# RoboEden/flatland-marl

Hardware: AMD Instinct MI355X
Metric: agent-steps/sec (batched envs) + tree-obs build ms/step (higher is better)
Workload: dtype int32; 1 GPU; cfg2: 256 envs x 30x30 / 20 agents / 3 cities (Round-2 Test_2); envs_per_gpu=256, agents=20, obs=cutils(31 nodes, pred 500) + upstream tree depth 2 (pred 30), actions=counter-hash uniform 0..4 generated on device, auto-reset at episode end, distinct_maps=8, dm_rebuild=at commit only, parallelism=envs sharded over 1 GPU(s), metrics all-reduce only, launch=one host call per kernel launch

## Files before the change

### flatland_marl_amd/csrc/fl_obs_body.h

```cpp
#pragma once
#include "fl_obs_trees.h"

__device__ __forceinline__ int obs_env_of_workgroup(const FlObsScratch &S) { return __builtin_amdgcn_readfirstlane(S.order ? S.order[blockIdx.x] : (int)blockIdx.x); }

template <bool CUTILS, int VAR, int STAGE, int MERGED = 0, int FIX = 0, bool UP = true>
__device__ __forceinline__ void obs_body(const FlDev &d, const FlObsScratch &S, const ObsArgs &P_launch) {
    using FixT = ObsFixed<FIX != 0 ? FIX : 1>;
    ObsArgs P_local = P_launch;
    if (FIX != 0) {
        P_local.max_nodes = FixT::max_nodes; P_local.pred_depth = FixT::pred_depth; P_local.tree_pred = FixT::shape.tree_pred;
        P_local.tshift = obs_fixed_tshift<FIX != 0 ? FIX : 1>(d.A);
        if (FixT::max_depth != 0) {
            P_local.max_depth = FixT::max_depth;
            P_local.n_tree_nodes = FixT::max_depth == 2 ? 21 : 85;
        }
    }
    const ObsArgs &P = P_local;
    constexpr bool TAB_LDS = (VAR & 1) != 0, WL_HBM = (VAR & 2) != 0;
    const int b = MERGED == 1 ? (int)blockIdx.x : obs_env_of_workgroup(S), tid = threadIdx.x,
              nt = MERGED == 3 ? 512 : (FIX != 0 || MERGED == 1 || MERGED == 2) ? OBS_NT : (int)blockDim.x;
    const int A = (FIX != 0 && FixT::agents != 0) ? FixT::agents : d.A, R = d.R[b], NS = R * 4, K = d.K[b], U = d.U[b];
    const int Rcap = d.Rcap, Scap = Rcap * 4;
    const int lane = tid & 63, wave = tid >> 6;

// ... 590 lines not shown
                    cutils_pass_a<OBS_CAP_C, TEAM>(X, d, P, b, team_id, have, grp, gl,
                                  merged ? merged_table_c(wave_scr, min(team_id, ROUND - 1)) : wave_scr + min(team_id, min((nt >> 6) * 2, A)) * (N_WORDS_C * OBS_CAP_C),
                                  a_vpos, a_pos, a_dir, a_state, a_speed, a_tslot, (float)T,
                                  a_raw ? a_raw[(have ? team_id : 0) * 8 + 1] : d.spk[b * A + (have ? team_id : 0)],
                                  a_raw ? a_raw[(have ? team_id : 0) * 8 + 2] : d.malf[b * A + (have ? team_id : 0)], node_base, levels);
                    if (gl == 0 && have) { team_meta[64 + team_id] = node_base; team_meta[192 + team_id] = levels; }
                };
                if (p_compact_t) hoisted(std::integral_constant<int, 16>());
                else hoisted(std::integral_constant<int, 32>());
            }
#ifdef FL_OBS_TIMING
            if (lane == 0) {
                atomicMax((unsigned long long *)&X.dbg[19], (unsigned long long)wall_clock64());
                atomicMax((unsigned long long *)&X.dbg[23], (unsigned long long)((long long)wall_clock64() - t_pa0));
            }
#endif
            drain_jobs();
        }
#ifdef FL_OBS_TIMING
        if (lane == 0) atomicMax((unsigned long long *)&X.dbg[22], (unsigned long long)wall_clock64());
#endif
        if (bk && !bk_lds) {
            __syncthreads();
            for (int i = wave; i < A; i += (nt >> 6)) {
                if (lab && lab[i] < 0) continue;
                const uint16_t *path = S.path + ((size_t)b * A + i) * OBS_PRED_CAP;
                const int lp = a_lp[i];
                const int tpc = a_tpc[i], tlast = X.Tn - 1;
                for (int k0 = lane; k0 <= lp; k0 += 256) {
                    uint32_t wv[4];
#pragma unroll
                    for (int q = 0; q < 4; q++) wv[q] = path[min(k0 + 64 * q, lp)];
#pragma unroll
                    for (int q = 0; q < 4; q++) {
                        const int k = k0 + 64 * q;
                        if (k > lp) break;
                        const int key = key_of(X, (int)(wv[q] >> 2));
                        const int tlo = k == 0 ? 0 : (k - 1) * tpc + 1, span = k == 0 ? 1 : tpc;
                        const int thi = (k == lp || tlo + span - 1 >= tlast) ? tlast : tlo + span - 1;
                        const int b1 = min(tlo >> bk_shift, bk_nb - 1), b2 = min(thi >> bk_shift, bk_nb - 1);
                        for (int bb = b1; bb <= b2; bb++) {
                            const int kb = bb * (K + 1) + key + 1;
                            atomicAdd(&bkc[kb >> 1], (kb & 1) ? 0x10000u : 1u);
                        }
                    }
                }
            }
        }
        } else if (!reuse) {
            for (int i = tid; i < A; i += nt) {
                const int n_c = a_n[i];
                const int n_py = (n_c - 1 < pred_depth) ? n_c : pred_depth;
                const int horizon = (X.Tn - 1) / a_tpc[i];
                a_lp[i] = (uint16_t)max(0, min(n_py - 1, horizon));
            }
            __syncthreads();
            for (int i = wave; i < A; i += (nt >> 6)) {
                const uint16_t *path = S.path + ((size_t)b * A + i) * OBS_PRED_CAP;
                const int lp = a_lp[i];
                for (int k = lane; k <= lp; k += 64) atomicAdd(&csr[key_of(X, (int)(path[k] >> 2))], 1);
            }
        }
        __syncthreads();
        OBS_STAMP(3);
        const bool bk_major = bk && !bk_lds;
        if (!reuse && !bk_major) {
            const int chunk = (K + 1 + nt - 1) / nt;
            const int lo = min(tid * chunk, K + 1), hi = min(lo + chunk, K + 1);
            int sum = 0;
            int longest = 0;
            for (int k = lo; k < hi; k++) {
                sum += dual ? (csr[k] | (csr2[k] << 16)) : csr[k];
                longest = max(longest, dual ? max(csr[k], csr2[k]) : csr[k]);
            }
            if (longest > CF_DIRECT && !bk) misc[11] = 1;
            partial[tid] = sum;
            __syncthreads();
            if (wave == 0) {
                constexpr int PER = OBS_NT / 64;
                const int per = nt >> 6;
                int loc[PER], tot = 0;
#pragma unroll
                for (int q = 0; q < PER; q++) { loc[q] = q < per ? partial[lane * per + q] : 0; tot += loc[q]; }
                int incl = tot;
#pragma unroll
                for (int off = 1; off < 64; off <<= 1) { const int v = __shfl_up(incl, off); if (lane >= off) incl += v; }
                int run = incl - tot;
#pragma unroll
                for (int q = 0; q < PER; q++) { if (q < per) partial[lane * per + q] = run; run += loc[q]; }
            }
            __syncthreads();
            int run = partial[tid];
            if (dual) {
                for (int k = lo; k < hi; k++) {
                    const int v = csr[k] | (csr2[k] << 16);
                    csr[k] = run & 0xFFFF; csr2[k] = (int)((unsigned)run >> 16);
                    run += v;
                }
                if (hi == K + 1 && lo < hi) { misc[2] = run & 0xFFFF; misc[3] = (int)((unsigned)run >> 16); }
            } else {
                for (int k = lo; k < hi; k++) { const int v = csr[k]; csr[k] = run; run += v; }
                if (hi == K + 1 && lo < hi) misc[2] = run;
            }
        }
        if (bk_major) {
            uint16_t *c16 = reinterpret_cast<uint16_t *>(bkc);
            const int K1 = K + 1, n = K1 * bk_nb;
            {
                int most = 0;
                for (int key = tid; key < K; key += nt) {
                    int prev = 0;
                    for (int bb = 0; bb < bk_nb; bb++) { const int c = c16[bb * K1 + key + 1]; most = max(most, prev + c); prev = c; }
                }
                if (most > CF_DIRECT) misc[11] = 1;
            }
            const int chunk = (n + nt - 1) / nt;
            const int lo = min(tid * chunk, n), hi = min(lo + chunk, n);
            int sum = 0;
            for (int k = lo; k < hi; k++) sum += c16[k];
            partial[tid] = sum;
            __syncthreads();
            if (wave == 0) {
                constexpr int PER = OBS_NT / 64;
                const int per = nt >> 6;
                int loc[PER], tot = 0;
#pragma unroll
                for (int q = 0; q < PER; q++) { loc[q] = q < per ? partial[lane * per + q] : 0; tot += loc[q]; }
                int incl = tot;
#pragma unroll
                for (int off = 1; off < 64; off <<= 1) { const int v = __shfl_up(incl, off); if (lane >= off) incl += v; }
                int run = incl - tot;
#pragma unroll
                for (int q = 0; q < PER; q++) { if (q < per) partial[lane * per + q] = run; run += loc[q]; }
            }
            __syncthreads();
            {
                int run = partial[tid];
                for (int k = lo; k < hi; k++) {
                    if (k % K1 == 0) misc[12 + k / K1] = run;
                    run += c16[k];
                }
                if (hi == n && lo < hi) misc[2] = run;
            }
            __syncthreads();
            {
                int run = partial[tid], row = lo / K1, rbase = lo < n ? misc[12 + row] : 0, next = (row + 1) * K1;
                for (int k = lo; k < hi; k++) {
                    if (k == next) { row++; rbase = misc[12 + row]; next += K1; }
                    const int c = c16[k];
                    c16[k] = (uint16_t)(run - rbase);
                    run += c;
                }
            }
        }
        __syncthreads();
        if (reuse) {
            csr = csr2; X.csr_end = csr2; X.items_lds = items2;
            X.tmask = p_use_tmask ? tmaskb : nullptr;
            if (!X.tmask) { X.wl_occ_cap = wl_entries; X.wl_cf = X.wl_occ + X.wl_occ_cap; X.wl_cf_cap = 0; }
        }
        if (bk_lds) {
            for (int key = tid; key < K; key += nt) {
                uint32_t *w4 = bkc + key * (bk_w / 2);
                uint32_t run = 0, prev = 0, most = 0;
                for (int q = 0; q < bk_nb / 2; q++) {
                    const uint32_t v = w4[q], c0 = v & 0xFFFFu, c1 = v >> 16;
                    most = max(most, max(prev + c0 + c1, c0 + c1));
                    prev = c0 + c1;
                    w4[q] = run | ((run + c0) << 16);
                    run += c0 + c1;
                }
                if (bk_lds) {
                    const uint32_t ve = w4[bk_nb / 2];
                    w4[bk_nb / 2] = run | (ve & 0xFFFF0000u);
                    most += ve & 0xFFFFu;
                }
                if (most > CF_DIRECT) misc[11] = 1;
            }
            __syncthreads();
        }
#ifdef FL_OBS_TIMING
        if (STAGE != 2) { __syncthreads(); if (tid == 0) P.dbg[(size_t)b * 64 + 56] = (long long)wall_clock64(); }
#endif
        const bool fit = items_lds != nullptr && misc[2] <= L_FIELD(items_cap);
        const bool dual_fill = dual && misc[3] <= L_FIELD(items2_cap);
        if (dual && tid == 0) misc[4] = dual_fill ? 1 : 0;
        if (merged && UP && !dual_fill) atomicCAS(&d.err[b], 0, FL_ERR_CAPACITY);
        if (fit && !reuse) { csr_items = items_lds; X.items_lds = items_lds; }
        constexpr int FU = 4;
#ifdef OBS_NO_LEAN_FILL
        constexpr bool LEAN_FILL = false;
#else
        constexpr bool LEAN_FILL = MERGED == 1;
#endif
        uint32_t pfv[FU] = {0, 0, 0, 0}, pfn[FU] = {0, 0, 0, 0}, pfp[FU] = {0, 0, 0, 0};
        auto prefetch = [&](int ia) __attribute__((always_inline)) {
            if (reuse || ia >= A) return;
            const uint16_t *pth = S.path + ((size_t)b * A + ia) * OBS_PRED_CAP;
            const int lpn = a_lp[ia];
#pragma unroll
            for (int q = 0; q < FU; q++) {
                const int k = min(lane + 64 * q, lpn);
                pfv[q] = pth[k]; pfn[q] = pth[min(k + 1, lpn)]; pfp[q] = pth[max(k - 1, 0)];
            }
        };
        if (bk_major) {
            const int K1 = K + 1, tlast = X.Tn - 1;
            uint16_t *pre16 = reinterpret_cast<uint16_t *>(partial);
            uint16_t *klo16 = pre16 + ((A + 2) & ~1);
            for (int bb = 0; bb < bk_nb; bb++) {
                const int t0 = bb << bk_shift, t1 = bb == bk_nb - 1 ? tlast : min(t0 + (1 << bk_shift) - 1, tlast);
                if (t0 > tlast) break;
                const int gbase = misc[12 + bb];
                for (int ia = tid; ia < A; ia += nt) {
                    const int lp = a_lp[ia], tpc = a_tpc[ia];
                    const int k_lo = min((t0 + tpc - 1) / tpc, lp);
                    const int k_hi = min(t1 >= 1 ? (t1 - 1) / tpc + 1 : 0, lp);
                    klo16[ia] = (uint16_t)k_lo;
                    pre16[ia + 1] = (lab && lab[ia] < 0) ? (uint16_t)0 : (uint16_t)(k_hi - k_lo + 1);
                }
                if (tid == 0) pre16[0] = 0;
                __syncthreads();
                if (wave == 0) {
                    const int per = (A + 63) >> 6, a_lo = min(lane * per, A), a_hi = min(a_lo + per, A);
                    int sum = 0;
                    for (int ia = a_lo; ia < a_hi; ia++) sum += pre16[ia + 1];
                    int incl = sum;
#pragma unroll
                    for (int off = 1; off < 64; off <<= 1) { const int v = __shfl_up(incl, off); if (lane >= off) incl += v; }
                    int run = incl - sum;
                    for (int ia = a_lo; ia < a_hi; ia++) { run += pre16[ia + 1]; pre16[ia + 1] = (uint16_t)run; }
                }
                __syncthreads();
                const int total = pre16[A];
                uint32_t nv = 0, nn = 0, np = 0;
                int n_i = 0, n_k = 0;
                auto request = [&](int t) __attribute__((always_inline)) {
                    if (t >= total) return;
                    int lo_a = 0, hi_a = A - 1;
                    while (lo_a < hi_a) {
                        const int mid = (lo_a + hi_a + 1) >> 1;
                        if ((int)pre16[mid] <= t) lo_a = mid; else hi_a = mid - 1;
                    }
                    n_i = lo_a;
                    n_k = (int)klo16[lo_a] + (t - (int)pre16[lo_a]);
                    const uint16_t *pth = S.path + ((size_t)b * A + lo_a) * OBS_PRED_CAP;
                    const int lp = a_lp[lo_a];
                    nv = pth[n_k]; nn = pth[min(n_k + 1, lp)]; np = pth[max(n_k - 1, 0)];
                };
                request(tid);
                for (int t = tid; t < total; t += nt) {
                    const int i = n_i, k = n_k;
                    const uint32_t w = nv, wnx = nn, wpv = np;
                    request(t + nt);
                    const int lp = a_lp[i], tpc = a_tpc[i];
                    const int tlo = k == 0 ? 0 : (k - 1) * tpc + 1, span = k == 0 ? 1 : tpc;
                    const bool to_end = k == lp || tlo + span - 1 >= tlast;
                    const int thi = to_end ? tlast : tlo + span - 1;
                    const int b1 = min(tlo >> bk_shift, bk_nb - 1), b2 = min(thi >> bk_shift, bk_nb - 1);
                    if (bb < b1 || bb > b2) continue;
                    const int key = key_of(X, (int)(w >> 2));
                    if (X.tmask && bb == b1) {
                        const int m1 = tb_of(tlo, X.tshift), m2 = tb_of(thi, X.tshift);
                        atomicOr(&tmask[key], ((2ull << m2) - 1ull) & ~((1ull << m1) - 1ull));
                    }
                    const uint32_t dnext = k < lp ? (wnx & 3u) : (w & 3u), dprev = k > 0 ? (wpv & 3u) : (w & 3u);
                    const uint32_t item = IT_MAKE(lab ? (int)lab[i] : i, tlo, to_end, span, dprev, dnext, w & 3u);
                    const int kb = bb * K1 + key + 1;
                    const uint32_t old = atomicAdd(&bkc[kb >> 1], (kb & 1) ? 0x10000u : 1u);
                    csr_items[gbase + (int)((kb & 1) ? (old >> 16) : (old & 0xFFFFu))] = item;
                }
                __syncthreads();
            }
        }
        prefetch(bk_major ? A : wave);
        for (int i = wave; !reuse && !bk_major && i < A; i += (nt >> 6)) {
            const uint16_t *path = S.path + ((size_t)b * A + i) * OBS_PRED_CAP;
            const int lp = (lab && lab[i] < 0) ? -1 : (int)a_lp[i], tpc = a_tpc[i], tlast = X.Tn - 1;
            const int lp2 = dual_fill ? (int)a_lp2[i] : -1, tpc2 = dual_fill ? (int)a_tpc2[i] : 1;
            uint32_t wv[FU], wnx[FU], wpv[FU];
#pragma unroll
            for (int q = 0; q < FU; q++) { wv[q] = pfv[q]; wnx[q] = pfn[q]; wpv[q] = pfp[q]; }
            prefetch(i + (nt >> 6));
            for (int k0 = lane; k0 <= lp; k0 += 64 * FU) {
            if (k0 != lane) {
#pragma unroll
                for (int q = 0; q < FU; q++) {
                    const int k = min(k0 + 64 * q, lp);
                    wv[q] = path[k]; wnx[q] = path[min(k + 1, lp)]; wpv[q] = path[max(k - 1, 0)];
                }
            }
#pragma unroll
            for (int q = 0; q < FU; q++) {
                const int k = k0 + 64 * q;
                if (k > lp) break;
                const uint32_t w = wv[q];
                const uint32_t dnext = k < lp ? (wnx[q] & 3u) : (w & 3u), dprev = k > 0 ? (wpv[q] & 3u) : (w & 3u);
                int tlo, span;
                if (CUTILS) {
                    tlo = k == 0 ? 0 : (k - 1) * tpc + 1;
                    span = k == 0 ? 1 : tpc;
                } else {
                    tlo = k * tpc;
                    span = tpc;
                }
                const bool to_end = k == lp || tlo + span - 1 >= tlast;
                const int key = key_of(X, (int)(w >> 2));
                if (LEAN_FILL) {
                    const int b1 = tb_of(tlo, X.tshift), b2 = tb_of(to_end ? tlast : tlo + span - 1, X.tshift);
                    const unsigned long long bits = ((2ull << b2) - 1ull) & ~((1ull << b1) - 1ull);
                    const bool second = k <= lp2, done = a_state[i] == ST_DONE;
                    const int tlo2 = k * tpc2, tlast2 = Tn2 - 1;
                    const bool to_end2 = k == lp2 || tlo2 + tpc2 - 1 >= tlast2;
// ... 199 lines not shown
```

### flatland_marl_amd/csrc/fl_obs_ctx.h

```cpp
#pragma once
#include <stdio.h>
#include <type_traits>

#include "../../include/flatland_hip.h"
#include "fl_obs_layout.h"

struct ObsCtx {
    int A, R;
    int SS;
    const uint32_t *cellw;
    const uint16_t *nbr;
    const uint16_t *snext;
    const uint16_t *rkey;
    const int *slot_agent;
    const int *slot_ready;
    const uint32_t *cell_target;
    const uint16_t *a_vpos;
    const uint8_t *a_dir, *a_state;
    const uint16_t *a_malf;
    const double *a_speed;
    const uint16_t *a_tpc;
    const double *a_tq;
    const uint16_t *a_tslot;
    const uint16_t *a_target;
    const uint16_t *a_srank;
    const int *csr_end;
    const uint32_t *items_lds;
    const uint32_t *items_glb;
    const uint16_t *bk_rel_lds;
    int bk_nb, bk_shift;
    const uint16_t *bk_rel;
    const int *bk_base;
    int bk_k1;
    int Tn;
    const uint16_t *dm;
    const uint4 *seg;
    uint2 *wl_occ, *wl_cf;
    int wl_occ_cap, wl_cf_cap;
    uint2 *wl_head_occ, *wl_head_cf;
    int wl_head_occ_n, wl_head_cf_n;
    int *wl_cnt;
    const int *long_lists;
    const unsigned long long *tmask;
    int tshift;
    int n_cu;
    int round_base;
    const int *u_csr_end;
    const uint32_t *u_items;
    const unsigned long long *u_tmask;
    int u_Tn, u_tshift;
    const double *a_tq2;
    const unsigned long long *tmask_m2, *u_tmask_m2;
    const unsigned long long *cmask;
    const uint32_t *u_cmask;
    bool pb_ceil_split;
#ifdef FL_OBS_COUNTS
    bool cf_count_only;
#endif
    const uint16_t *path;
    int pred_cap;
    const uint16_t *a_lp, *a_lp2, *a_tpc2;
    long long *dbg;
    int dbg_base;
};

#ifndef OBS_NT_LEVEL
#define OBS_NT_LEVEL 2
#endif
typedef float obs_f4_t __attribute__((ext_vector_type(4)));
typedef double obs_d2_t __attribute__((ext_vector_type(2)));
__device__ __forceinline__ void fill_store_d2(double *p, double a, double b) {
#if OBS_NT_LEVEL >= 1
    const obs_d2_t v = {a, b};
    __builtin_nontemporal_store(v, reinterpret_cast<obs_d2_t *>(p));
#else
    *reinterpret_cast<double2 *>(p) = make_double2(a, b);
#endif
}
__device__ __forceinline__ void out_store_f4(float *p, float a, float b, float c, float d) {
#if OBS_NT_LEVEL >= 2
    const obs_f4_t v = {a, b, c, d};
    __builtin_nontemporal_store(v, reinterpret_cast<obs_f4_t *>(p));
#else
    *reinterpret_cast<float4 *>(p) = make_float4(a, b, c, d);
#endif
}
__device__ __forceinline__ void out_store_d2(double *p, double a, double b) {
#if OBS_NT_LEVEL >= 2
    const obs_d2_t v = {a, b};
    __builtin_nontemporal_store(v, reinterpret_cast<obs_d2_t *>(p));
#else
    *reinterpret_cast<double2 *>(p) = make_double2(a, b);
#endif
}

template <typename T>
__device__ __forceinline__ void out_store(T *p, T v) {
#if OBS_NT_LEVEL >= 3
    __builtin_nontemporal_store(v, p);
#else
    *p = v;
#endif
}

__device__ __forceinline__ int tb_of(int t, int ts) { return min(t >> ts, 63); }

__device__ __forceinline__ uint32_t cw_bits(const ObsCtx &X, int r) { return X.cellw[r] & 0xFFFFu; }
__device__ __forceinline__ uint32_t cw_slot(const ObsCtx &X, int r) { return X.cellw[r] >> 16; }
__device__ __forceinline__ uint32_t cw_load(const ObsCtx &X, int r) { return X.cellw[r]; }
__device__ __forceinline__ int key_of(const ObsCtx &X, int r) { return X.rkey ? (int)X.rkey[r] : r; }
__device__ __forceinline__ uint32_t cf_against(uint32_t cd) { return 1u << (3u - ((cd + 2u) & 3u)); }
__device__ __forceinline__ uint32_t cf_dirs_of(uint32_t bits16, uint32_t against, bool done) {
    uint32_t dirs = 0;
#pragma unroll
    for (uint32_t d = 0; d < 4; d++) {
        const uint32_t nib = nibble(bits16, d);
        if (nib != 0 && (done || (nib & against & ~cf_against(d)) != 0)) dirs |= 1u << d;
    }
    return dirs;
}
__device__ __forceinline__ uint32_t cf_dirs_swar(uint32_t bits16, uint32_t against, bool done) {
    const uint32_t x = done ? bits16 : (bits16 & (against * 0x1111u) & 0xDE7Bu);
    uint32_t y = x | (x >> 1);
    y = (y | (y >> 2)) & 0x1111u;
    return ((y * 0x8421u) >> 12) & 15u;
}
template <int PB>
__device__ __forceinline__ bool pb_cu(const ObsCtx &X, int team) { return PB == 3 ? true : PB == 2 ? team < X.n_cu : PB == 1; }
template <int PB>
__device__ __forceinline__ int pb_handle(const ObsCtx &X, const int *team_meta, int team) {
    return PB == 3 ? X.round_base + team : PB == 2 ? X.round_base + (team < X.n_cu ? team : team - X.n_cu) : team_meta[128 + team];
}
template <int PB>
__device__ __forceinline__ int pt_of(const ObsCtx &X, bool cu, int handle, int tot) {
    if (PB == 2 && !cu) return (int)((double)tot * X.a_tq2[handle]);
    return cu ? (int)((float)tot * (float)X.a_tq[handle]) : (int)((double)tot * X.a_tq[handle]);
}
struct ListRange { int lo, n1, lo2, n; };
template <bool TWO>
__device__ __forceinline__ int list_index(const ListRange &R, int v) { return (TWO && v >= R.n1) ? R.lo2 + (v - R.n1) : R.lo + v; }
template <int PB>
__device__ __forceinline__ ListRange list_range(const ObsCtx &X, bool cu, int r, int pt) {
    const int key = key_of(X, r);
    ListRange R;
    R.lo2 = 0;
    if (PB == 2 && !cu) {
        R.lo = key > 0 ? X.u_csr_end[key - 1] : 0;
        R.n1 = R.n = X.u_csr_end[key] - R.lo;
// ... 107 lines not shown
```

### flatland_marl_amd/csrc/fl_obs_passb.h

```cpp
#pragma once
#include "fl_obs_ctx.h"
#include "fl_obs_slices.h"

__device__ __forceinline__ void occ_event(const ObsCtx &X, bool CUTILS, int *sc, int cap, int node, uint32_t sl, uint32_t d, int tot) {
    const int ag = X.slot_agent[sl];
    if (ag < 0) return;
    atomicMin(&nt_w(sc, cap, N_OA, node), tot);
    const int mf = (int)X.a_malf[ag];
    if (mf > 0) {
        if (CUTILS) atomicOr(&nt_w(sc, cap, N_RM, node), 1 << 16);
        else atomicMax(&nt_w(sc, cap, N_MALF, node), mf);
    }
    const int rd = X.slot_ready[sl];
    const int radd = rd > 0 ? (CUTILS ? rd - 1 : rd) : 0;
    if (radd) atomicAdd(&nt_w(sc, cap, N_RM, node), radd);
    if (X.a_dir[ag] == d) {
        atomicAdd(&nt_w(sc, cap, N_CNT, node), 1);
        const double sp = CUTILS ? (double)(float)X.a_speed[ag] : X.a_speed[ag];
        if (sp < 1.0) atomicMin(reinterpret_cast<unsigned int *>(&nt_w(sc, cap, N_MS, node)), ((unsigned int)X.a_srank[ag] << 10) | (unsigned int)ag);
    } else {
        atomicAdd(&nt_w(sc, cap, N_CNT, node), 1 << 16);
    }
}

// ... 66 lines not shown

__device__ __forceinline__ uint2 wl_occ_get(const ObsCtx &X, int i) { return i < X.wl_head_occ_n ? X.wl_head_occ[i] : X.wl_occ[i]; }
__device__ __forceinline__ void wl_occ_put(const ObsCtx &X, int i, uint2 e) { if (i < X.wl_head_occ_n) X.wl_head_occ[i] = e; else X.wl_occ[i] = e; }
__device__ __forceinline__ uint2 wl_cf_get(const ObsCtx &X, int i) { return i < X.wl_head_cf_n ? X.wl_head_cf[i] : X.wl_cf[i]; }
__device__ __forceinline__ void wl_cf_put(const ObsCtx &X, int i, uint2 e) { if (i < X.wl_head_cf_n) X.wl_head_cf[i] = e; else X.wl_cf[i] = e; }
__device__ __forceinline__ void wl_cf_set_y(const ObsCtx &X, int i, uint32_t y) { if (i < X.wl_head_cf_n) X.wl_head_cf[i].y = y; else X.wl_cf[i].y = y; }
__device__ __forceinline__ uint32_t wl_cf_done(const ObsCtx &X, int i, uint32_t bits) {
    if (i < X.wl_head_cf_n) {
        if (bits) atomicOr(&X.wl_head_cf[i].y, bits);
        return atomicSub(&X.wl_head_cf[i].y, 1u << 9);
    }
    if (bits) atomicOr(&X.wl_cf[i].y, bits);
    return atomicSub(&X.wl_cf[i].y, 1u << 9);
}

__device__ __forceinline__ bool wl_push_cf(const ObsCtx &X, bool want, uint2 e) {
    const unsigned long long m = __ballot(want);
    if (m == 0) return true;
    const int lane = (int)__lane_id();
    int base = 0;
    if (lane == __ffsll((long long)__ballot(1)) - 1) base = atomicAdd(&X.wl_cnt[1], __popcll(m));
    base = __builtin_amdgcn_readfirstlane(base);
    const int idx = base + __popcll(m & ((1ull << lane) - 1ull));
    if (want && idx < X.wl_cf_cap) wl_cf_put(X, idx, e);
    return !want || idx < X.wl_cf_cap;
}

__device__ __forceinline__ unsigned long long wl_reserve2_issue(int *cnt, unsigned long long m0, unsigned long long m1) {
    unsigned long long old = 0;
    int zero;
    asm volatile("v_mov_b32 %0, 0" : "=v"(zero));
    if ((m0 | m1) != 0ull && (int)__lane_id() == __ffsll((long long)__ballot(1)) - 1)
        old = atomicAdd(reinterpret_cast<unsigned long long *>(cnt) + zero, (unsigned long long)__popcll(m0) | ((unsigned long long)__popcll(m1) << 32));
    return old;
}
__device__ __forceinline__ void wl_reserve2_finish(unsigned long long old, unsigned long long m0, unsigned long long m1, int &i0, int &i1) {
    const int b0 = __builtin_amdgcn_readfirstlane((int)(uint32_t)old), b1 = __builtin_amdgcn_readfirstlane((int)(uint32_t)(old >> 32));
    const unsigned long long lt = (1ull << __lane_id()) - 1ull;
    i0 = b0 + __popcll(m0 & lt);
    i1 = b1 + __popcll(m1 & lt);
}

#ifdef FL_OBS_TIMING
#define WAVE_MARK(X, k, k2) do { if ((X).dbg && (threadIdx.x & 63) == 0) { const long long now_ = (long long)wall_clock64() & 0xFFFFFFFFFFll; \
    atomicMax((unsigned long long *)&(X).dbg[(X).dbg_base + (k)], (unsigned long long)now_); \
    if ((k2) >= 0) atomicMax((unsigned long long *)&(X).dbg[(X).dbg_base + ((k2) < 0 ? 0 : (k2))], (unsigned long long)((1ll << 40) - now_)); } } while (0)
#else
#define WAVE_MARK(X, k, k2) do {} while (0)
#endif
#ifdef FL_OBS_TIMING
#define WL_ACC(X, k) do { if ((X).dbg && (threadIdx.x & 63) == 0) atomicAdd((unsigned long long *)&(X).dbg[(k) == 5 ? 48 : 51 + (k)], (unsigned long long)((long long)wall_clock64() - wl_t0_)); } while (0)
#else
#define WL_ACC(X, k) do {} while (0)
#endif
#ifdef FL_OBS_TIMING
#define TREE_STAMP(X, k) do { __syncthreads(); if (threadIdx.x == 0 && (X).dbg) { const long long now_ = (long long)wall_clock64(); (X).dbg[(X).dbg_base + (k)] += now_ - (X).dbg[(X).dbg_base + 15]; (X).dbg[(X).dbg_base + 15] = now_; } } while (0)
#else
#define TREE_STAMP(X, k) do {} while (0)
#endif

__device__ __forceinline__ void team_sync() {
    __builtin_amdgcn_fence(__ATOMIC_RELEASE, "wavefront");
    __builtin_amdgcn_wave_barrier();
    __builtin_amdgcn_fence(__ATOMIC_ACQUIRE, "wavefront");
}

template <int TEAM, int CAP, bool UPSTREAM, int STRIDE = CAP>
__device__ __forceinline__ int team_prepare(bool have, int tl, int n_nodes, int *scr, int &first_real) {
    constexpr int NCH = (CAP + TEAM - 1) / TEAM;
    const int tbase = ((int)__lane_id() / TEAM) * TEAM;
    const unsigned long long tbits = TEAM == 64 ? ~0ull : ((1ull << (TEAM & 63)) - 1ull);
    int v[NCH];
    unsigned long long real[NCH];
#pragma unroll
    for (int c = 0; c < NCH; c++) {
        const int k = c * TEAM + tl;
        v[c] = (have && k < n_nodes && k < CAP) ? nt_vis((uint32_t)nt_r(scr, STRIDE, N_TV, k)) : 0;
        real[c] = (__ballot(v[c] > 0) >> tbase) & tbits;
    }
    int run_base = 0;
#pragma unroll
    for (int c = 0; c < NCH; c++) {
        const int k = c * TEAM + tl;
        int incl = v[c];
#pragma unroll
        for (int off = 1; off < TEAM; off <<= 1) { const int u = __shfl_up(incl, off, TEAM); if (tl >= off) incl += u; }
        incl += run_base;
        int nxt = 0xFF;
#pragma unroll
        for (int c2 = NCH - 1; c2 > c; c2--)
            if (real[c2]) nxt = c2 * TEAM + __ffsll((long long)real[c2]) - 1;
        const unsigned long long above = tl + 1 < TEAM ? real[c] >> ((tl + 1) & 63) : 0ull;
        if (above) nxt = k + __ffsll((long long)above);
        if (k < CAP) {
            nt_w(scr, STRIDE, N_INCL, k) = incl | (nxt << 24);
            nt_w(scr, STRIDE, N_OA, k) = 0x7fffffff; nt_w(scr, STRIDE, N_PC, k) = 0x7fffffff;
            nt_w(scr, STRIDE, N_CNT, k) = 0; nt_w(scr, STRIDE, N_RM, k) = 0;
            nt_w(scr, STRIDE, N_MS, k) = -1;
            if (UPSTREAM) { nt_w(scr, STRIDE, N_OT, k) = 0x7fffffff; nt_w(scr, STRIDE, N_MALF, k) = 0; }
        }
        run_base = __shfl(incl, TEAM - 1, TEAM);
    }
    first_real = 0xFF;
#pragma unroll
    for (int c = NCH - 1; c >= 0; c--)
        if (real[c]) first_real = c * TEAM + __ffsll((long long)real[c]) - 1;
    return run_base;
}

template <int PB, int CAP>
__device__ __forceinline__ int *team_table(const ObsCtx &X, int *scr0, int team_words, int team) {
    if (PB == 3) return scr0 + team * (N_WORDS_C * 32);
    if (PB == 2) {
        const int u = team - X.n_cu;
        return u < 0 ? scr0 + team * (N_WORDS_C * 32) : scr0 + X.n_cu * (N_WORDS_C * 32) + (u >> 1) * (N_WORDS_T * 32) + (u & 1) * 16;
    }
    return scr0 + team * team_words;
}

template <int PB, int CAP>
__device__ __forceinline__ bool cf_settled(const ObsCtx &X, int *scr0, int team_words, int team, int node, int tot) {
#ifdef OBS_NO_PC_SKIP
    return false;
#else
    constexpr int cap = PB >= 2 ? 32 : CAP;
    return nt_r(team_table<PB, CAP>(X, scr0, team_words, team), cap, N_PC, node) <= tot;
#endif
}

struct NoLateWork { __device__ __forceinline__ void operator()() const {} };

template <int PB, int CAP, bool ITL, typename LATE = NoLateWork, bool TWO = false>
__device__ __forceinline__ void wg_pass_b(const ObsCtx &X, int tid, int nt, int n_teams, int *scr0, int team_words,
                                          const int *team_meta, const LATE &late = LATE()) {
    if (tid == 0) { X.wl_cnt[0] = 0; X.wl_cnt[1] = 0; X.wl_cnt[2] = 0; }
    __syncthreads();
    const int lane = tid & 63;
    const int tv = lane < n_teams ? team_meta[lane] : 0;
    int tincl = tv;
#pragma unroll
    for (int off = 1; off < 64; off <<= 1) { const int u = __shfl_up(tincl, off); if (lane >= off) tincl += u; }
    const int total = __builtin_amdgcn_readlane(tincl, 63);
    const PbSplit split = pb_split(total, nt, X.pb_ceil_split);
    int pos = pb_lane_begin(split, tid);
    const int end = pb_lane_end(split, tid);
    const int wv = __builtin_amdgcn_readfirstlane(tid >> 6);
    const int wpos0 = pb_wave_first(split, wv);
    int team = 0, t_excl = 0;
    if (wpos0 < total) {
        const int wlast = pb_wave_last(split, wv);
        int ulo = 0, uhi = n_teams - 1;
        while (ulo < uhi) {
            const int mid = (ulo + uhi) >> 1;
            if (__builtin_amdgcn_readlane(tincl, mid) > wpos0) uhi = mid; else ulo = mid + 1;
        }
        team = ulo;
        t_excl = ulo > 0 ? __builtin_amdgcn_readlane(tincl, ulo - 1) : 0;
        const int ppos = min(pos, total - 1);
        for (int t = ulo; t < n_teams - 1; t++) {
            const int v = __builtin_amdgcn_readlane(tincl, t);
            if (v > wlast) break;
            if (ppos >= v) { team = t + 1; t_excl = v; }
        }
    }
#ifdef FL_OBS_TIMING
    const long long dbg_t1 = (long long)wall_clock64();
    int dbg_skip = 0;
    const int dbg_cells = end - pos;
#endif
#ifdef FL_OBS_COUNTS
    int cnt_iter = 0, cnt_switch = 0;
#endif
    if (pos < end) {
        constexpr int cap = PB >= 2 ? 32 : CAP;
        const int *vs = team_table<PB, CAP>(X, scr0, team_words, team);
        int nn = team_meta[64 + team];
        int handle = pb_handle<PB>(X, team_meta, team);
        const int lpos = pos - t_excl;
        int lo = 0, hi = nn - 1;
        while (lo < hi) {
            const int m2 = (lo + hi) >> 1, m1 = (lo + m2) >> 1, m3 = (m2 + 1 + hi) >> 1;
            const int i1 = nt_r(vs, cap, N_INCL, m1) & 0xFFFFFF, i2 = nt_r(vs, cap, N_INCL, m2) & 0xFFFFFF, i3 = nt_r(vs, cap, N_INCL, m3) & 0xFFFFFF;
            if (i1 > lpos) hi = m1;
            else if (i2 > lpos) { lo = m1 + 1; hi = m2; }
            else if (i3 > lpos) { lo = m2 + 1; hi = m3; }
            else lo = min(m3 + 1, hi);
        }
        int node = lo;
        int target;
        double tq;
        bool cu;
        const unsigned long long *tmask_t = X.tmask, *tmask2_t = X.tmask_m2;
        int Tn_t = X.Tn, tshift_t = X.tshift;
        const bool self_filter = PB >= 2 && X.tmask_m2 != nullptr;
        const uint16_t *path_t = X.path;
        int lp_t = 0, tpc_t = 1;
        const bool cf_any = PB >= 2 && (X.cmask != nullptr || X.u_cmask != nullptr);
        bool cf_t = false;
        auto enter_team = [&]() __attribute__((always_inline)) {
            target = X.a_target[handle];
            cu = pb_cu<PB>(X, team);
            tq = (PB == 2 && !cu) ? X.a_tq2[handle] : X.a_tq[handle];
            if (PB == 2) { tmask_t = cu ? X.tmask : X.u_tmask; Tn_t = cu ? X.Tn : X.u_Tn; tshift_t = cu ? X.tshift : X.u_tshift; }
            if (PB >= 2 && self_filter) {
                tmask2_t = cu ? X.tmask_m2 : X.u_tmask_m2;
                path_t = X.path + (size_t)handle * X.pred_cap;
                lp_t = cu ? X.a_lp[handle] : X.a_lp2[handle];
                tpc_t = cu ? X.a_tpc[handle] : X.a_tpc2[handle];
            }
            if (PB >= 2 && cf_any) cf_t = cu ? X.cmask != nullptr : X.u_cmask != nullptr;
        };
        enter_team();
        int left, cell, tot, nxt;
        uint32_t dd;
        {
            const uint32_t inw = (uint32_t)nt_r(vs, cap, N_INCL, node), tvw = (uint32_t)nt_r(vs, cap, N_TV, node);
            const int nvis = nt_vis(tvw), incl = (int)(inw & 0xFFFFFFu);
            const int k = lpos - (incl - nvis);
            const uint32_t st = skip_cells(X, (uint32_t)nt_r(vs, cap, N_SE, node) & 0xFFFFu, k);
            cell = (int)(st >> 2); dd = st & 3u;
#ifdef FL_OBS_TIMING
            dbg_skip = k;
#endif
            tot = nt_tot(tvw) + k;
// ... 108 lines not shown
            cnt_iter++;
            cnt_switch += __ballot(cnt_moved) != 0ull;
#endif
            int i_occ, i_cf;
            wl_reserve2_finish(resv, m_occ, m_cf, i_occ, i_cf);
            if (occ) {
                if (i_occ < X.wl_occ_cap) wl_occ_put(X, i_occ, entry);
                else occ_event(X, e_cu, sc, e_cap, e_node, sl, e_dd, e_tot);
            }
            if (to_cf) {
                if (i_cf < X.wl_cf_cap) wl_cf_put(X, i_cf, entry);
                else conflict_event<PB, ITL, TWO>(X, e_cu, sc, e_cap, e_node, e_handle, e_cell, e_dd, e_tot, pt);
            } else if (cand) {
                conflict_event<PB, ITL, TWO>(X, e_cu, sc, e_cap, e_node, e_handle, e_cell, e_dd, e_tot, pt);
            }
            if (tgt_hit) atomicMin(&nt_w(sc, e_cap, N_OT, e_node), e_tot);
            if (!more) break;
        }
        };
        if (PB >= 2 || (X.tmask != nullptr && X.snext != nullptr && X.rkey == nullptr)) walk(std::true_type());
        else walk(std::false_type());
    }
#ifdef FL_OBS_TIMING
    if (X.dbg && lane == 0) {
        const long long dbg_t2 = (long long)wall_clock64();
        atomicMax((unsigned long long *)&X.dbg[25], ((unsigned long long)(dbg_t2 - dbg_t1) << 40) | ((unsigned long long)dbg_cells << 20) | (unsigned long long)dbg_skip);
        atomicMax((unsigned long long *)&X.dbg[26], (unsigned long long)total);
    }
#endif
#ifdef FL_OBS_COUNTS
    if (X.dbg && lane == 0 && X.dbg_base == 0) {
        atomicAdd((unsigned long long *)&X.dbg[44], (unsigned long long)cnt_iter);
        atomicAdd((unsigned long long *)&X.dbg[45], (unsigned long long)cnt_switch);
        if (wpos0 >= total) atomicAdd((unsigned long long *)&X.dbg[47], 1ull);
        if (tid == 0) atomicMax((unsigned long long *)&X.dbg[49], ((unsigned long long)split.q << 20) | (unsigned long long)split.rem);
    }
#endif
    __syncthreads();
    TREE_STAMP(X, 11);
    WAVE_MARK(X, 18, -1);
#ifdef FL_OBS_TIMING
    const long long wl_t0_ = (long long)wall_clock64();
#endif
    const int n_occ = min(X.wl_cnt[0], X.wl_occ_cap), n_cf = min(X.wl_cnt[1], X.wl_cf_cap);
#ifdef FL_OBS_TIMING
    if (X.dbg && tid == 0) { X.dbg[X.dbg_base + 9] += n_occ; X.dbg[X.dbg_base + 10] += n_cf; }
#endif
    for (int e = tid; e < n_occ; e += nt) {
        const uint2 w = wl_occ_get(X, e);
        const int cell = (int)((w.x & 0xFFFFFFu) >> 2), team = (int)(w.x >> 24);
        constexpr int cap = PB >= 2 ? 32 : CAP;
        int *sc = team_table<PB, CAP>(X, scr0, team_words, team);
        occ_event(X, pb_cu<PB>(X, team), sc, cap, (int)(w.y >> 24), cw_slot(X, cell), w.x & 3u, (int)(w.y & 0xFFFFFFu));
    }
    WAVE_MARK(X, 12, -1);
    WL_ACC(X, 0);
    if (*X.long_lists == 0) {
        for (int e = tid; e < n_cf; e += nt) {
            const uint2 w = wl_cf_get(X, e);
            const int cell = (int)((w.x & 0xFFFFFFu) >> 2), team = (int)(w.x >> 24);
            const int handle = pb_handle<PB>(X, team_meta, team), tot = (int)(w.y & 511u);
            if (cf_settled<PB, CAP>(X, scr0, team_words, team, (int)(w.y >> 24), tot)) continue;
            const bool cu = pb_cu<PB>(X, team);
            const int pt = pt_of<PB>(X, cu, handle, tot);
            const ListRange R = list_range<PB>(X, cu, cell, pt);
#ifdef FL_OBS_COUNTS
            const uint32_t f = R.n > 0 ? conflict_flags<PB, ITL, TWO>(X, cu, handle, cell, w.x & 3u, pt, R, 0, R.n) : 0u;
            if (X.dbg) {
                atomicAdd((unsigned long long *)&X.dbg[X.dbg_base + 27], (unsigned long long)R.n);
                if (tb_of(pt, X.tshift) >= 63) atomicAdd((unsigned long long *)&X.dbg[X.dbg_base + 28], 1ull);
                if (f & 7u) atomicAdd((unsigned long long *)&X.dbg[X.dbg_base + 29], 1ull);
                if (conflict_hit(f)) atomicAdd((unsigned long long *)&X.dbg[X.dbg_base + 30], 1ull);
                if (!(f & 7u) && (f & 64u)) atomicAdd((unsigned long long *)&X.dbg[X.dbg_base + 31], 1ull);
            }
            if (conflict_hit(f)) {
#else
            if (R.n > 0 && conflict_hit(conflict_flags<PB, ITL, TWO>(X, cu, handle, cell, w.x & 3u, pt, R, 0, R.n))) {
#endif
                constexpr int cap = PB >= 2 ? 32 : CAP;
                int *sc = team_table<PB, CAP>(X, scr0, team_words, team);
                atomicMin(&nt_w(sc, cap, N_PC, (int)(w.y >> 24)), tot);
            }
        }
        WAVE_MARK(X, 13, 17);
        WL_ACC(X, 1);
        late();
        WL_ACC(X, 2);
        __syncthreads();
        WL_ACC(X, 5);
        return;
    }
    constexpr int CF_CHUNK = ITL ? CF_CHUNK_LDS : CF_CHUNK_HBM;
    constexpr int CF_FIRST = ITL ? CF_CHUNK_LDS : CF_FIRST_HBM;
    for (int e0 = 0; e0 < n_cf; e0 += nt) {
        const int e = e0 + tid;
        int nch = 0, cell = 0, handle = 0, tot = 0, pt = 0, team = 0, np = 0;
        ListRange R = {0, 0, 0, 0};
        bool cu = PB == 1;
        uint2 w = make_uint2(0u, 0u);
        uint32_t fl = 0;
        if (e < n_cf) {
            w = wl_cf_get(X, e);
            cell = (int)((w.x & 0xFFFFFFu) >> 2);
            team = (int)(w.x >> 24);
            handle = pb_handle<PB>(X, team_meta, team);
            tot = (int)(w.y & 511u);
            cu = pb_cu<PB>(X, team);
            pt = pt_of<PB>(X, cu, handle, tot);
            R = list_range<PB>(X, cu, cell, pt);
            if (cf_settled<PB, CAP>(X, scr0, team_words, team, (int)(w.y >> 24), tot)) R.n = 0;
            nch = 1 + min(max(R.n - CF_FIRST + CF_CHUNK - 1, 0) / CF_CHUNK, 62);
            const uint32_t f = R.n > 0 ? conflict_flags<PB, ITL, TWO>(X, cu, handle, cell, w.x & 3u, pt, R, 0, min(R.n, CF_FIRST)) : 0u;
#ifdef FL_OBS_COUNTS
            if (X.dbg) {
                atomicAdd((unsigned long long *)&X.dbg[X.dbg_base + 27], (unsigned long long)R.n);
                if (tb_of(pt, X.tshift) >= 63) atomicAdd((unsigned long long *)&X.dbg[X.dbg_base + 28], 1ull);
                if (f & 7u) atomicAdd((unsigned long long *)&X.dbg[X.dbg_base + 29], 1ull);
                if (conflict_hit(f)) atomicAdd((unsigned long long *)&X.dbg[X.dbg_base + 30], 1ull);
                if (!(f & 7u) && (f & 64u)) atomicAdd((unsigned long long *)&X.dbg[X.dbg_base + 31], 1ull);
            }
#endif
            fl = f & 63u;
        }
        for (int j = 1; __any(j < nch); j++) {
            const bool want = j < nch;
            if (!wl_push_cf(X, want, make_uint2(w.x, (uint32_t)j | ((uint32_t)e << 6) | ((uint32_t)tot << 23)))) {
                fl |= conflict_flags<PB, ITL, TWO>(X, cu, handle, cell, w.x & 3u, pt, R, CF_FIRST + (j - 1) * CF_CHUNK, j == 62 ? R.n : min(R.n, CF_FIRST + j * CF_CHUNK)) & 63u;
            } else if (want) np++;
        }
        if (e < n_cf) {
            if (np == 0) {
                if (conflict_hit(fl)) {
                    constexpr int cap = PB >= 2 ? 32 : CAP;
                    int *sc = team_table<PB, CAP>(X, scr0, team_words, team);
                    atomicMin(&nt_w(sc, cap, N_PC, (int)(w.y >> 24)), tot);
                }
            } else {
                wl_cf_set_y(X, e, w.y | ((uint32_t)np << 9) | (fl << 15));
            }
        }
    }
    WAVE_MARK(X, 13, 17);
    WL_ACC(X, 1);
    late();
    WL_ACC(X, 2);
    __syncthreads();
    WAVE_MARK(X, 14, -1);
    WL_ACC(X, 3);
    const int n_cf2 = min(X.wl_cnt[1], X.wl_cf_cap);
    for (int e = n_cf + tid; e < n_cf2; e += nt) {
        const uint2 w = wl_cf_get(X, e);
        const int cell = (int)((w.x & 0xFFFFFFu) >> 2), team = (int)(w.x >> 24);
        const int first = (int)((w.y >> 6) & 0x1FFFFu), chunk = (int)(w.y & 63u), tot = (int)(w.y >> 23);
        const int handle = pb_handle<PB>(X, team_meta, team);
        const bool cu = pb_cu<PB>(X, team);
        const int pt = pt_of<PB>(X, cu, handle, tot);
        const ListRange R = list_range<PB>(X, cu, cell, pt);
        const bool settled = cf_settled<PB, CAP>(X, scr0, team_words, team, (int)(wl_cf_get(X, first).y >> 24), tot);
        const uint32_t f = settled ? 0u : conflict_flags<PB, ITL, TWO>(X, cu, handle, cell, w.x & 3u, pt, R, CF_FIRST + (chunk - 1) * CF_CHUNK, chunk == 62 ? R.n : min(R.n, CF_FIRST + chunk * CF_CHUNK));
        const uint32_t old = wl_cf_done(X, first, (f & 63u) << 15);
        if (((old >> 9) & 63u) == 1u && conflict_hit((old >> 15) & 63u)) {
            constexpr int cap = PB >= 2 ? 32 : CAP;
            int *sc = team_table<PB, CAP>(X, scr0, team_words, team);
            atomicMin(&nt_w(sc, cap, N_PC, (int)(old >> 24)), (int)(old & 511u));
        }
    }
    WL_ACC(X, 4);
    WL_ACC(X, 5);
    __syncthreads();
}
```

### flatland_marl_amd/csrc/fl_obs_trees.h

```cpp
#pragma once
#include "fl_obs_passb.h"

template <bool CUTILS>
__device__ __forceinline__ void node_row(const ObsCtx &X, int handle, const int *scr, int cap, int k, double *f) {
    const uint32_t tv = (uint32_t)nt_r(scr, cap, N_TV, k), uf = (uint32_t)nt_r(scr, cap, N_UF, k);
    const int tot_end = nt_tot(tv) + nt_vis(tv) - 1;
    const uint32_t flags = nt_flags(uf);
    const bool tgt = flags & ND_TARGET;
    double dist_min = 0;
    if (flags & ND_PHANTOM) dist_min = INFINITY;
    else if (!tgt) {
        const uint16_t dv = X.dm[X.a_tslot[handle] * X.SS + nt_end((uint32_t)nt_r(scr, cap, N_SE, k))];
        dist_min = dv == FL_INF16 ? INFINITY : (double)dv;
    }
    const int oa = nt_r(scr, cap, N_OA, k), pc = nt_r(scr, cap, N_PC, k), ot = CUTILS ? 0x7fffffff : nt_r(scr, cap, N_OT, k), un = nt_unus(uf);
    const uint32_t cnt = (uint32_t)nt_r(scr, cap, N_CNT, k), rm = (uint32_t)nt_r(scr, cap, N_RM, k), ms = (uint32_t)nt_r(scr, cap, N_MS, k);
    f[0] = tgt ? (double)tot_end : INFINITY;
    f[1] = ot == 0x7fffffff ? INFINITY : (double)ot;
    f[2] = oa == 0x7fffffff ? INFINITY : (double)oa;
    f[3] = pc == 0x7fffffff ? INFINITY : (double)pc;
    f[4] = un < 0 ? INFINITY : (double)un;
    f[5] = (flags & ND_TERMINAL) ? INFINITY : (double)tot_end;
    f[6] = dist_min;
    f[7] = (double)(cnt & 0xFFFFu); f[8] = (double)(cnt >> 16);
// ... 364 lines not shown
                                             const uint16_t *a_vpos, const int *a_pos, const uint8_t *a_dir,
                                             const uint8_t *a_state, const double *a_speed, const uint16_t *a_tslot,
                                             float max_dist, bool hoisted) {
    constexpr int CAP = TC, TW = N_WORDS_C * TC, TPW = 64 / TC;
    const int A = X.A;
    const int grp = TC == 64 ? 0 : lane >> 5, gl = lane & (TC - 1);
    int *scr = wave_scr + min(wave * TPW + grp, min(nwaves * TPW, A)) * TW;
    for (int base = 0; base < A; base += nwaves * TPW) {
        const int i = base + wave * TPW + grp;
        const bool have = i < A;
        int node_base, levels;
        if (hoisted && base == 0) {
            node_base = team_meta[64 + wave * TPW + grp];
            levels = team_meta[192 + wave * TPW + grp];
        } else {
            cutils_pass_a<TC>(X, d, P, b, i, have, grp, gl, scr, a_vpos, a_pos, a_dir, a_state, a_speed, a_tslot, max_dist,
                              d.spk[b * A + (have ? i : 0)], d.malf[b * A + (have ? i : 0)], node_base, levels);
        }
        TREE_STAMP(X, 6);
        {
            int first;
            const int tot_cells = team_prepare<TC, CAP, false>(have, gl, have ? node_base : 1, scr, first);
            const int team_id = wave * TPW + grp;
            if (gl == 0) { team_meta[team_id] = have ? tot_cells : 0; team_meta[64 + team_id] = have ? node_base : 1; team_meta[128 + team_id] = have ? i : -1; team_meta[256 + team_id] = first; }
        }
        wg_pass_b<1, CAP, ITL, NoLateWork, !ITL>(X, wave * 64 + lane, nwaves * 64, nwaves * TPW, wave_scr, TW, team_meta);
        TREE_STAMP(X, 7);
        cutils_rows_orders<TC, I64>(X, d, P, b, i, have, gl, scr, node_base, levels, max_dist);
        team_sync();
        TREE_STAMP(X, 16);
    }
}

__device__ __forceinline__ int *merged_table_c(int *wave_scr, int t) { return wave_scr + t * (N_WORDS_C * 32); }
template <int ROUND>
__device__ __forceinline__ int *merged_table_t(int *wave_scr, int u) {
    return wave_scr + ROUND * (N_WORDS_C * 32) + (u >> 1) * (N_WORDS_T * 32) + (u & 1) * 16;
}
template <int ROUND>
__device__ __forceinline__ int merged_upstream_of(int wave, int lane, int nwaves) {
    const int u = (nwaves - 1 - wave) * 4 + (lane >> 4);
    return u < ROUND ? u : -1;
}

template <bool ITL, bool MULTI, int ROUND, bool UP, typename LATE>
__device__ __forceinline__ void trees_merged(ObsCtx &X, const FlDev &d, const ObsArgs &P, int b, int wave, int lane, int nwaves,
                                             int *wave_scr, int *team_meta, const uint16_t *a_vpos, const int *a_pos, const uint8_t *a_dir,
                                             const uint8_t *a_state, const double *a_speed, const uint16_t *a_tslot, float max_dist,
                                             const LATE &late, uint4 *rowmask) {
    constexpr int CT = OBS_CAP_T_COMPACT;
    const int A = X.A;
    const int grp = lane >> 5, gl = lane & 31, ct = wave * 2 + grp;
    int *scr_c = merged_table_c(wave_scr, min(ct, ROUND - 1));
    const int u = UP ? merged_upstream_of<ROUND>(wave, lane, nwaves) : -1, tl = lane & 15;
    const bool wave_has_u = UP && (nwaves - 1 - wave) * 4 < ROUND;
    int *scr_u = merged_table_t<ROUND>(wave_scr, u < 0 ? 0 : u);
    const int ns = upstream_slots<true>(P);
    for (int base = 0; base < (MULTI ? A : 1); base += ROUND) {
        X.round_base = base;
        const int i_c = base + ct, i_u = base + u;
        const bool have_c = ct < ROUND && i_c < A, have_u = u >= 0 && i_u < A;
        int node_base = 1, levels = 0;
        if (!MULTI || base == 0) {
            if (have_c) { node_base = team_meta[64 + ct]; levels = team_meta[192 + ct]; }
        } else {
            if (ct < ROUND)
                cutils_pass_a(X, d, P, b, i_c, have_c, grp, gl, scr_c, a_vpos, a_pos, a_dir, a_state, a_speed, a_tslot, max_dist,
                              d.spk[b * A + (have_c ? i_c : 0)], d.malf[b * A + (have_c ? i_c : 0)], node_base, levels);
            if (wave_has_u) upstream_pass_a<16, CT, true, 32>(X, P, b, i_u, have_u, tl, scr_u, &d.err[b]);
        }
        TREE_STAMP(X, 6);
        if (ct < ROUND) {
            int first;
            const int cells = team_prepare<32, OBS_CAP_C, false>(have_c, gl, have_c ? node_base : 1, scr_c, first);
            if (gl == 0) { team_meta[ct] = have_c ? cells : 0; team_meta[64 + ct] = have_c ? node_base : 1; team_meta[192 + ct] = levels; team_meta[256 + ct] = first; }
        }
        if (wave_has_u) {
            int first;
            const int cells = team_prepare<16, CT, true, 32>(have_u, tl, have_u ? ns : 1, scr_u, first);
            const int id = ROUND + (u < 0 ? 0 : u);
            if (u >= 0 && tl == 0) { team_meta[id] = have_u ? cells : 0; team_meta[64 + id] = have_u ? ns : 1; team_meta[256 + id] = first; }
        }
        wg_pass_b<UP ? 2 : 3, OBS_CAP_C, ITL, LATE, MULTI>(X, wave * 64 + lane, nwaves * 64, UP ? 2 * ROUND : ROUND, wave_scr, 0, team_meta, late);
        if (base == 0) late();
        TREE_STAMP(X, 7);
        if (MULTI || !OBS_TOPO_JOBS) {
            if (ct < ROUND) cutils_rows_orders<OBS_CAP_C, !UP>(X, d, P, b, i_c, have_c, gl, scr_c, node_base, levels, max_dist);
            if (wave_has_u) upstream_rows<16, CT, true, 32>(X, P, b, i_u, have_u, tl, scr_u, rowmask);
        } else {
            if (ct < ROUND) cutils_rows_orders<OBS_CAP_C, !UP, 2>(X, d, P, b, i_c, have_c, gl, scr_c, node_base, levels, max_dist);
            if (wave_has_u) upstream_rows<16, CT, true, 32>(X, P, b, i_u, have_u, tl, scr_u, rowmask);
            TREE_STAMP(X, 8);
            late(true);
        }
        team_sync();
        TREE_STAMP(X, 16);
    }
}
```

Baseline: 126.4 million agent-steps/s.

## Use DPP wave scans and restructure pass-B control flow around long lists

Replaces the shfl_up-based inclusive prefix scans in several places with a DPP row_shr/row_bcast sequence (wave_incl_scan), which cuts the LDS-backed shuffle traffic. It also restructures wg_pass_b so the short-list branch falls through to shared tail code and returns early only when no long lists exist. It further removes an extra late() call after wg_pass_b in the tree driver. The DPP bcast masks must be correct for a 64-lane wavefront, and the segmented TEAM scans lose their width argument, which risks incorrect results if TEAM segments do not align with rows.

```diff
diff --git a/flatland_marl_amd/csrc/fl_obs_body.h b/flatland_marl_amd/csrc/fl_obs_body.h
--- a/flatland_marl_amd/csrc/fl_obs_body.h
+++ b/flatland_marl_amd/csrc/fl_obs_body.h
@@ -696,9 +696,7 @@
                 int loc[PER], tot = 0;
 #pragma unroll
                 for (int q = 0; q < PER; q++) { loc[q] = q < per ? partial[lane * per + q] : 0; tot += loc[q]; }
-                int incl = tot;
-#pragma unroll
-                for (int off = 1; off < 64; off <<= 1) { const int v = __shfl_up(incl, off); if (lane >= off) incl += v; }
+                const int incl = wave_incl_scan<64>(tot);
                 int run = incl - tot;
 #pragma unroll
                 for (int q = 0; q < PER; q++) { if (q < per) partial[lane * per + q] = run; run += loc[q]; }
@@ -740,9 +738,7 @@
                 int loc[PER], tot = 0;
 #pragma unroll
                 for (int q = 0; q < PER; q++) { loc[q] = q < per ? partial[lane * per + q] : 0; tot += loc[q]; }
-                int incl = tot;
-#pragma unroll
-                for (int off = 1; off < 64; off <<= 1) { const int v = __shfl_up(incl, off); if (lane >= off) incl += v; }
+                const int incl = wave_incl_scan<64>(tot);
                 int run = incl - tot;
 #pragma unroll
                 for (int q = 0; q < PER; q++) { if (q < per) partial[lane * per + q] = run; run += loc[q]; }
@@ -839,10 +835,7 @@
                     const int per = (A + 63) >> 6, a_lo = min(lane * per, A), a_hi = min(a_lo + per, A);
                     int sum = 0;
                     for (int ia = a_lo; ia < a_hi; ia++) sum += pre16[ia + 1];
-                    int incl = sum;
-#pragma unroll
-                    for (int off = 1; off < 64; off <<= 1) { const int v = __shfl_up(incl, off); if (lane >= off) incl += v; }
-                    int run = incl - sum;
+                    int run = wave_incl_scan<64>(sum) - sum;
                     for (int ia = a_lo; ia < a_hi; ia++) { run += pre16[ia + 1]; pre16[ia + 1] = (uint16_t)run; }
                 }
                 __syncthreads();
diff --git a/flatland_marl_amd/csrc/fl_obs_ctx.h b/flatland_marl_amd/csrc/fl_obs_ctx.h
--- a/flatland_marl_amd/csrc/fl_obs_ctx.h
+++ b/flatland_marl_amd/csrc/fl_obs_ctx.h
@@ -64,6 +64,18 @@
     int dbg_base;
 };
 
+template <int W>
+__device__ __forceinline__ int wave_incl_scan(int v) {
+    static_assert(W == 16 || W == 32 || W == 64, "segments of 16, 32 or 64 lanes");
+    v += __builtin_amdgcn_update_dpp(0, v, 0x111, 0xf, 0xf, false);
+    v += __builtin_amdgcn_update_dpp(0, v, 0x112, 0xf, 0xf, false);
+    v += __builtin_amdgcn_update_dpp(0, v, 0x114, 0xf, 0xf, false);
+    v += __builtin_amdgcn_update_dpp(0, v, 0x118, 0xf, 0xf, false);
+    if (W >= 32) v += __builtin_amdgcn_update_dpp(0, v, 0x142, 0xa, 0xf, false);
+    if (W >= 64) v += __builtin_amdgcn_update_dpp(0, v, 0x143, 0xc, 0xf, false);
+    return v;
+}
+
 #ifndef OBS_NT_LEVEL
 #define OBS_NT_LEVEL 2
 #endif
diff --git a/flatland_marl_amd/csrc/fl_obs_passb.h b/flatland_marl_amd/csrc/fl_obs_passb.h
--- a/flatland_marl_amd/csrc/fl_obs_passb.h
+++ b/flatland_marl_amd/csrc/fl_obs_passb.h
@@ -172,10 +172,7 @@
 #pragma unroll
     for (int c = 0; c < NCH; c++) {
         const int k = c * TEAM + tl;
-        int incl = v[c];
-#pragma unroll
-        for (int off = 1; off < TEAM; off <<= 1) { const int u = __shfl_up(incl, off, TEAM); if (tl >= off) incl += u; }
-        incl += run_base;
+        int incl = wave_incl_scan<TEAM>(v[c]) + run_base;
         int nxt = 0xFF;
 #pragma unroll
         for (int c2 = NCH - 1; c2 > c; c2--)
@@ -227,9 +224,7 @@
     __syncthreads();
     const int lane = tid & 63;
     const int tv = lane < n_teams ? team_meta[lane] : 0;
-    int tincl = tv;
-#pragma unroll
-    for (int off = 1; off < 64; off <<= 1) { const int u = __shfl_up(tincl, off); if (lane >= off) tincl += u; }
+    const int tincl = wave_incl_scan<64>(tv);
     const int total = __builtin_amdgcn_readlane(tincl, 63);
     const PbSplit split = pb_split(total, nt, X.pb_ceil_split);
     int pos = pb_lane_begin(split, tid);
@@ -504,14 +499,7 @@
                 atomicMin(&nt_w(sc, cap, N_PC, (int)(w.y >> 24)), tot);
             }
         }
-        WAVE_MARK(X, 13, 17);
-        WL_ACC(X, 1);
-        late();
-        WL_ACC(X, 2);
-        __syncthreads();
-        WL_ACC(X, 5);
-        return;
-    }
+    } else {
     constexpr int CF_CHUNK = ITL ? CF_CHUNK_LDS : CF_CHUNK_HBM;
     constexpr int CF_FIRST = ITL ? CF_CHUNK_LDS : CF_FIRST_HBM;
     for (int e0 = 0; e0 < n_cf; e0 += nt) {
@@ -562,11 +550,17 @@
             }
         }
     }
+    }
     WAVE_MARK(X, 13, 17);
     WL_ACC(X, 1);
     late();
     WL_ACC(X, 2);
     __syncthreads();
+    if (*X.long_lists == 0) {
+        WL_ACC(X, 5);
+        return;
+    }
+    constexpr int CF_CHUNK = ITL ? CF_CHUNK_LDS : CF_CHUNK_HBM, CF_FIRST = ITL ? CF_CHUNK_LDS : CF_FIRST_HBM;
     WAVE_MARK(X, 14, -1);
     WL_ACC(X, 3);
     const int n_cf2 = min(X.wl_cnt[1], X.wl_cf_cap);
diff --git a/flatland_marl_amd/csrc/fl_obs_trees.h b/flatland_marl_amd/csrc/fl_obs_trees.h
--- a/flatland_marl_amd/csrc/fl_obs_trees.h
+++ b/flatland_marl_amd/csrc/fl_obs_trees.h
@@ -470,7 +470,6 @@
             if (u >= 0 && tl == 0) { team_meta[id] = have_u ? cells : 0; team_meta[64 + id] = have_u ? ns : 1; team_meta[256 + id] = first; }
         }
         wg_pass_b<UP ? 2 : 3, OBS_CAP_C, ITL, LATE, MULTI>(X, wave * 64 + lane, nwaves * 64, UP ? 2 * ROUND : ROUND, wave_scr, 0, team_meta, late);
-        if (base == 0) late();
         TREE_STAMP(X, 7);
         if (MULTI || !OBS_TOPO_JOBS) {
             if (ct < ROUND) cutils_rows_orders<OBS_CAP_C, !UP>(X, d, P, b, i_c, have_c, gl, scr_c, node_base, levels, max_dist);
```

Result: faster. 130.8 million agent-steps/s (median of 6 runs) (+3.5%).
